# vwxyzjn/cleanrl

Measured on NVIDIA H100. Metric: env steps/sec (SPS) PPO Breakout num_envs=1024, higher is better.
Workload: dtype bf16

## Files before the change

cleanrl_b200/csrc/net_impala_tc.cu:

```cuda
#include <cuda.h>
#include <algorithm>
#include <cstring>
#include "tc_base.cuh"
#include "tc_gemm_tma.cuh"
#include "tc_reduce.cuh"
#include "tc_heads.cuh"
#include "tc_mma_sync.cuh"

namespace b200rl {
using namespace tc;

namespace imp {

constexpr int kThreads = 256;
constexpr int kWgradCtas = 264;

__device__ __forceinline__ float bf_lo(uint32_t w) { return __uint_as_float(w << 16); }
__device__ __forceinline__ float bf_hi(uint32_t w) { return __uint_as_float(w & 0xFFFF0000u); }
__device__ __forceinline__ uint32_t relu2(uint32_t w) {
    const uint32_t neg = ((w >> 15) & 0x00010001u) * 0xFFFFu;
    return w & ~neg;
}

struct Geo {
// ... 658 lines not shown
    float* wssmall = reinterpret_cast<float*>(reinterpret_cast<uint8_t*>(workspace) + impala_big_bytes());
    int rc;
    {
        ProfScope ps(s, "heads_bwd", 4.0 * n * 256 * A1, (double)n * (1024 + 8 * A1));
        if ((rc = heads_bwd_weight<256>(dhead, T(Q.hid), n, A1, wssmall, grads + L.hw, grads + L.hb, s, "impala/heads_bwd"))) return rc;
        if ((rc = heads_bwd_data<256>(dhead, params + L.hw, ab + Q.mhid, n, A1, T(Q.dhid), s, "impala/heads_bwd",
                                      values == 2 ? A : -1))) return rc;
    }
    {
        ProfScope ps(s, "fc_wgrad", 2.0 * n * 256 * 2048, (double)n * (2048 + 256) * 2 + 256.0 * 2048 * 4);
        const int splits = launch_wgrad_tma(T(Q.dhid), 256, T(Q.h0), 2048, n, wsbig, s, "impala/fc_wgrad");
        if (splits < 0) return splits;
        tc_fold_fc<<<2048, 256, 0, s>>>(wsbig, splits, 256, 2048, 256, 2048, 32, 64, 1.f, grads + L.fcw);
        if ((rc = check_launch("impala/fc_fold"))) return rc;
        if ((rc = colsum(T(Q.dhid), n, 256, 256, wssmall, grads + L.fcb, s))) return rc;
    }
    {
        KGemmParams g;
        memset(&g, 0, sizeof(g));
        g.scale = 1.f; g.A = T(Q.dhid); g.M = n; g.nchunks = 4;
        g.Bw = P + L.pfcd; g.N = 2048; g.out = T(Q.ga); g.ldo = 2048;
        g.mask_bits = reinterpret_cast<const uint32_t*>(ab + Q.mh0);
        ProfScope ps(s, "fc_dgrad", 2.0 * n * 256 * 2048, (double)n * (2048 + 256) * 2 + 256.0 * 2048 * 2);
        if ((rc = launch_gemm_tma<128, 4>(g, s, "impala/fc_dgrad"))) return rc;
    }
    bf16* G = T(Q.ga);
    bf16* Gn = T(Q.gb);
    const int cin[3] = {3, 16, 32}, cout[3] = {16, 32, 32};
    for (int q = 2; q >= 0; --q) {
        const int H = kH[q], OH = H / 2, C = cout[q], k0 = q * 5;
        for (int blk = 1; blk >= 0; --blk) {
            const int kc0 = k0 + 1 + 2 * blk, kc1 = kc0 + 1;
            bf16* x = T(Q.s[q][blk]);
            bf16* y0 = T(Q.y[q][blk]);
            ProfScope ps(s, "impala_res_bwd", 4 * 2.0 * n * OH * OH * C * 9 * C, 0);
            WgradP w1 = wgrad_defaults(geo(OH), wsbig, wssmall);
            w1.x = y0; w1.dy = G;
            ConvP d1 = conv_defaults(geo(OH));
            d1.in = G; d1.w = P + L.pd[kc1]; d1.epi = E_DGRAD; d1.aux = y0; d1.out = T(Q.gy);
            WgradP w0 = wgrad_defaults(geo(OH), wsbig, wssmall);
            w0.x = x; w0.relu_in = 1; w0.dy = T(Q.gy);
            ConvP d0 = conv_defaults(geo(OH));
            d0.in = T(Q.gy); d0.w = P + L.pd[kc0]; d0.epi = E_DGRAD; d0.aux = x; d0.skipg = G; d0.out = Gn;
            if (C == 16) {
                if ((rc = run_wgrad<16, 16>(w1, n, 1.f, grads + L.cw[kc1], grads + L.cb[kc1], s, "impala/res_wgrad1"))) return rc;
                if ((rc = run_conv<16, 16>(d1, n, s, "impala/res_dgrad1"))) return rc;
                if ((rc = run_wgrad<16, 16>(w0, n, 1.f, grads + L.cw[kc0], grads + L.cb[kc0], s, "impala/res_wgrad0"))) return rc;
// ... 50 lines not shown
```

cleanrl_b200/csrc/net_tc.cu:

```cuda
#include <cuda.h>
#include <algorithm>
#include "tc_base.cuh"
#include "tc_conv_win.cuh"
#include "tc_conv1_u8.cuh"
#include "tc_gemm_tma.cuh"
#include "tc_wgrad_win.cuh"
#include "tc_reduce.cuh"
#include "tc_aux.cuh"
#include "tc_heads.cuh"
#include "tc_heads_wide.cuh"
#include "tc_lstm.cuh"

namespace b200rl {

struct NatureLayout {
    int A;
    int64_t c1w, c1b, c2w, c2b, c3w, c3b, fcw, fcb, hw, hb, total;
    int64_t w1f, w2f, w2dg, w3f, w3dg, wfcf, wfcdg, w1l, w1sc, packed_total;
    bool wide; int G; int64_t whf, whdg, hbp;
    int64_t wih, whh, bih, bhh, whhp;
    explicit NatureLayout(int A_) : A(A_), wih(-1), whh(-1), bih(-1), bhh(-1), whhp(-1) {
        int64_t o = 0;
        c1w = o; o += 32 * 4 * 8 * 8;  c1b = o; o += 32;
        c2w = o; o += 64 * 32 * 4 * 4; c2b = o; o += 64;
// ... 147 lines not shown
    return wide_dhead_bytes(n, L) + colsum_f32_ws(n, A1);
}

static int trunk_fwd(const NatureLayout& L, const NatureActs& Q, const float* params, const bf16* P, bf16* act, int64_t n,
                     cudaStream_t s) {
    int rc;
    KGemmParams p;
    WinParams wp;
    win_defaults(wp); win_conv2(wp, act + Q.act1, n);
    wp.Bw = P + L.w2f; wp.N = 64; wp.vH = 9; wp.vW = 9; wp.out_mode = WOUT_DENSE; wp.out = act + Q.act2;
    wp.bias = params + L.c2b; wp.relu = 1; wp.mask_out = reinterpret_cast<uint32_t*>(act + Q.m2);
    { ProfScope ps(s, "conv2_fwd", 2.0 * n * 81 * 64 * 512, (double)n * ((12800 + 5184) * 2 + 648));
      if ((rc = launch_conv_win_t<128, 2, 2, 4>(wp, s, "naturecnn/conv2"))) return rc; }
    win_defaults(wp); win_conv3(wp, act + Q.act2, n);
    wp.Bw = P + L.w3f; wp.N = 64; wp.vH = 7; wp.vW = 7; wp.out_mode = WOUT_DENSE; wp.out = act + Q.act3;
    wp.bias = params + L.c3b; wp.relu = 1; wp.mask_out = reinterpret_cast<uint32_t*>(act + Q.m3);
    { ProfScope ps(s, "conv3_fwd", 2.0 * n * 49 * 64 * 576, (double)n * ((5184 + 3136) * 2 + 392));
      if ((rc = launch_conv_win_t<128, 1, 4, 9>(wp, s, "naturecnn/conv3"))) return rc; }
    gemm_rowmajor(p, act + Q.act3, n, 49);
    p.Bw = P + L.wfcf; p.N = 512; p.out = act + Q.hid; p.ldo = 512; p.bias = params + L.fcb; p.relu = 1;
    p.mask_out = reinterpret_cast<uint32_t*>(act + Q.m4);
    { ProfScope ps(s, "fc_fwd", 2.0 * n * 512 * 3136, (double)n * (3136 + 512) * 2 + 512.0 * 3136 * 2);
      if (n <= 8192) { if ((rc = launch_gemm_tma<64, 6>(p, s, "naturecnn/fc"))) return rc; }
      else if ((rc = launch_gemm_tma<128, 4>(p, s, "naturecnn/fc"))) return rc; }
    return B200RL_OK;
}

static int trunk_bwd(const NatureLayout& L, const NatureActs& Q, const bf16* P, bf16* act, float* grads, int64_t n,
                     float* wsbig, float* wssmall, void* tail_ready_event, bool dact1_fused, cudaStream_t s) {
    int rc;
    KGemmParams p;
    {
        int splits;
        { ProfScope ps(s, "fc_wgrad", 2.0 * n * 512 * 3136, (double)n * (3136 + 512) * 2 + 512.0 * 3136 * 4);
          if ((splits = launch_wgrad_tma(act + Q.dhid, 512, act + Q.act3, 3136, n, wsbig, s, "naturecnn/fc_wgrad")) < 0) return splits; }
        { ProfScope ps(s, "wgrad_fold_bias", 0, 0);
          note_launches(1); tc_fold_fc<<<(unsigned)ceil_div((int64_t)512 * 3136, 256), 256, 0, s>>>(wsbig, splits, 512, 13 * 256, 512, 3136, 64, 49, 1.f, grads + L.fcw);
          if ((rc = colsum(act + Q.dhid, n, 512, 512, wssmall, grads + L.fcb, s))) return rc; }
        if (tail_ready_event) {
            cudaError_t e = cudaEventRecord(reinterpret_cast<cudaEvent_t>(tail_ready_event), s);
            if (e != cudaSuccess) return fail(B200RL_ERR_CUDA, "naturecnn_backward: cudaEventRecord: %s", cudaGetErrorString(e));
        }
        gemm_rowmajor(p, act + Q.dhid, n, 8);
        p.Bw = P + L.wfcdg; p.N = 3136; p.out = act + Q.dact3a; p.out2 = act + Q.dact3b; p.dual_dact3 = 1;
        p.ldo = 3136; p.mask_bits = reinterpret_cast<const uint32_t*>(act + Q.m3);
        { ProfScope ps(s, "fc_dgrad", 2.0 * n * 512 * 3136, (double)n * ((3136 + 512) * 2 + 392) + 512.0 * 3136 * 2);
          if ((rc = launch_gemm_tma<128, 4>(p, s, "naturecnn/fc_dgrad"))) return rc; }
    }
    WGradWinParams gw;
    WinParams wp;
    FoldWin fw;
    {
        wgw_defaults(gw);
        gw.X = act + Q.act2; gw.M = n * 81; gw.n = (int)n; gw.G = 81; gw.cpr = 1; gw.nslots = 10; gw.WRX = round8(128 + 20);
        for (int t = 0; t < 9; ++t) gw.shift[t] = (t / 3) * 9 + (t % 3);
        const int st[10] = {0, 1, 2, 3, 4, 5, 6, 7, 7, 8};
        for (int k = 0; k < 10; ++k) { gw.slot_tap[k] = st[k]; gw.slot_cc[k] = 0; }
        gw.Y = act + Q.dact3a; gw.ldy = 64; gw.ncolsY = 64;
        const WPlan pl = conv3_wgrad_plan(n);
        gw.rows_per_cta = pl.rows_per_cta; gw.ws = wsbig; gw.wsb = wssmall;
        { ProfScope ps(s, "conv3_wgrad", 2.0 * n * 49 * 64 * 576, (double)n * (5184 + 5184) * 2);
          if ((rc = launch_wgrad_win(gw, pl.splits, s, "naturecnn/conv3_wgrad"))) return rc; }
        memset(&fw, 0, sizeof(fw));
        fw.layer = 3; fw.S = pl.splits; fw.nslots = 10; fw.Cout = 64; fw.scale = 1.f; fw.bscale = 1.f;
        for (int k = 0; k < 10; ++k) { fw.slot_tap[k] = st[k]; fw.slot_skip[k] = (k == 8); }
        { ProfScope ps(s, "wgrad_fold_bias", 0, 0);
          fw.wsb = wssmall; fw.db = grads + L.c3b;
          tc_fold_win<<<(unsigned)ceil_div(640 * 64 + 64, 32), 256, 0, s>>>(wsbig, fw, grads + L.c3w);
          if ((rc = check_launch("naturecnn/conv3_fold"))) return rc; }
        win_defaults(wp);
// ... 28 lines not shown
        for (int a = 0; a < 2; ++a) for (int b = 0; b < 2; ++b) wp.shift[a * 2 + b] = (1 - a) * 11 + (1 - b);
        wp.WR = round8(128 + 12);
        wp.Bw = P + L.w2dg; wp.N = 128; wp.vH = 10; wp.vW = 10; wp.out_mode = WOUT_DACT1;
        wp.out = act + Q.dact1; wp.mask_bits = reinterpret_cast<const uint32_t*>(act + Q.m1);
        { ProfScope ps(s, "conv2_dgrad", 2.0 * n * 400 * 32 * 256, (double)n * ((7744 + 14112) * 2 + 1600));
          if ((rc = launch_conv_win<128, 1, 4, 4>(wp, s, "naturecnn/conv2_dgrad"))) return rc; }
    }
    return B200RL_OK;
}
static size_t trunk_big_bytes(int64_t n) {
    return std::max({wgrad_tma_bytes(n, 512, 3136), wgrad_win_bytes(conv3_wgrad_plan(n).splits, 10),
                     wgrad_win_bytes(conv2_wgrad_plan(n).splits, 8)});
}
static size_t trunk_small_bytes(int64_t n) {
    return std::max({colsum_ws(n, 512), wgrad_win_bias_bytes(conv3_wgrad_plan(n).splits),
                     wgrad_win_bias_bytes(conv2_wgrad_plan(n).splits)});
}

static int wide_head_fwd(const NatureLayout& L, const bf16* P, const bf16* hid, int64_t n, int A1, float* out, cudaStream_t s) {
    KGemmParams p;
    gemm_rowmajor(p, hid, n, 8);
    p.Bw = P + L.whf; p.N = L.G; p.bias = reinterpret_cast<const float*>(P + L.hbp);
    p.out_f32 = out; p.ldo = A1; p.ncols_f32 = A1;
    return launch_gemm_tma<128, 4>(p, s, "wide_heads");
}

static int wide_head_bwd(const NatureLayout& L, const bf16* P, const float* dhead, int64_t n, int A1, const bf16* hid, bf16* dhid,
                         const uint32_t* hid_bits, float* dW, float* db, float* wsbig, float* wssmall, cudaStream_t s) {
    int rc;
    KGemmParams p;
    bf16* dh16 = reinterpret_cast<bf16*>(wssmall);
    float* dbpart = reinterpret_cast<float*>(reinterpret_cast<char*>(wssmall) + wide_dhead_bytes(n, L));
    int cb = (int)ceil_div(n * L.G, 256); if (cb > num_sms() * 8) cb = num_sms() * 8;
    tc_head_dhead_bf16<<<cb, 256, 0, s>>>(dhead, n, A1, L.G, dh16);
    if ((rc = check_launch("wide_heads_dhead"))) return rc;
    if ((rc = colsum_f32(dhead, n, A1, dbpart, db, s))) return rc;
    const int splits = launch_wgrad_tma(dh16, L.G, hid, 512, n, wsbig, s, "wide_heads_wgrad");
    if (splits < 0) return splits;
    tc_fold_fc<<<(unsigned)ceil_div((int64_t)A1 * 512, 256), 256, 0, s>>>(wsbig, splits, L.G, 512, A1, 512, 512, 1, 1.f, dW);
    if ((rc = check_launch("wide_heads_wgrad"))) return rc;
    gemm_rowmajor(p, dh16, n, L.G / 64);
    p.Bw = P + L.whdg; p.N = 512; p.out = dhid; p.ldo = 512;
    p.mask_bits = hid_bits;
    if (n <= 8192) { if ((rc = launch_gemm_tma<64, 6>(p, s, "wide_heads_dgrad"))) return rc; }
    else if ((rc = launch_gemm_tma<128, 4>(p, s, "wide_heads_dgrad"))) return rc;
    return B200RL_OK;
}
}

extern "C" int64_t b200rl_naturecnn_param_count(int A) { return A >= 1 ? NatureLayout(A).total : -1; }
extern "C" int64_t b200rl_naturecnn_grad_tail_offset(int A) { return A >= 1 ? NatureLayout(A).fcw : -1; }
extern "C" size_t b200rl_naturecnn_bf16_packed_bytes(int A) { return head_ok(A) ? (size_t)NatureLayout(A).packed_total * 2 : 0; }
extern "C" size_t b200rl_naturecnn_bf16_acts_bytes(int64_t n, int obs_format) {
    return n >= 0 ? (size_t)NatureActs(n, obs_format == B200RL_OBS_U8_NCHW).total * 2 + 256 : 0;
}

extern "C" int b200rl_frames_to_s2d_bf16(const uint8_t* obs, const int64_t* rows, int64_t n, void* out, void* stream) {
    B200RL_REQUIRE(n >= 0, "frames_to_s2d: negative n");
    if (n == 0) return B200RL_OK;
    B200RL_REQUIRE(obs && out, "frames_to_s2d: null pointer");
    B200RL_REQUIRE(aligned(obs, 4) && aligned(out, 16), "frames_to_s2d: misaligned buffer");
    cudaStream_t s = (cudaStream_t)stream;
    ProfScope ps(s, "frames_to_s2d", 0, (double)n * 28224 * 3);
    tc_frames_to_s2d<<<(unsigned)ceil_div(n * 1764, 256), 256, 0, s>>>(obs, rows, n, reinterpret_cast<bf16*>(out));
    return check_launch("frames_to_s2d");
}

extern "C" int b200rl_frames_to_s2d_u8(const uint8_t* obs, const int64_t* rows, int64_t n, uint8_t* out_rm, uint8_t* out_cm, void* stream) {
// ... 367 lines not shown
```

cleanrl_b200/csrc/tc_common.cuh:

```cuda
#pragma once
#include <cuda_bf16.h>
#include <cstdint>
#include "tc_wgmma.cuh"

namespace b200rl { namespace tc {

__device__ __forceinline__ uint32_t smem_u32(const void* p) {
    return static_cast<uint32_t>(__cvta_generic_to_shared(p));
}

__device__ __forceinline__ void mbar_init(uint64_t* bar, uint32_t count) {
    asm volatile("mbarrier.init.shared::cta.b64 [%0], %1;" ::"r"(smem_u32(bar)), "r"(count) : "memory");
}
__device__ __forceinline__ void fence_barrier_init() {
    asm volatile("fence.mbarrier_init.release.cluster;" ::: "memory");
}
__device__ __forceinline__ bool mbar_try_wait(uint64_t* bar, uint32_t parity) {
    uint32_t ok;
    asm volatile(
        "{\n\t.reg .pred p;\n\t"
        "mbarrier.try_wait.parity.shared::cta.b64 p, [%1], %2;\n\t"
        "selp.u32 %0, 1, 0, p;\n\t}\n"
        : "=r"(ok)
        : "r"(smem_u32(bar)), "r"(parity)
// ... 71 lines not shown

__device__ __forceinline__ uint32_t pack_bf16x2_relu(float lo, float hi) {
    uint32_t d;
    asm("cvt.rn.relu.bf16x2.f32 %0, %1, %2;" : "=r"(d) : "f"(hi), "f"(lo));
    return d;
}
__device__ __forceinline__ uint32_t pack_bf16x2(float lo, float hi) {
    __nv_bfloat162 v = __floats2bfloat162_rn(lo, hi);
    return *reinterpret_cast<uint32_t*>(&v);
}

}}

namespace b200rl { namespace tc {
__device__ __forceinline__ void cp_async16(uint32_t smem_addr, const void* gptr, uint32_t src_bytes) {
    asm volatile("cp.async.cg.shared.global [%0], [%1], 16, %2;" ::"r"(smem_addr), "l"(gptr), "r"(src_bytes) : "memory");
}
__device__ __forceinline__ void cp_async_commit() { asm volatile("cp.async.commit_group;" ::: "memory"); }
template <int N>
__device__ __forceinline__ void cp_async_wait() { asm volatile("cp.async.wait_group %0;" ::"n"(N) : "memory"); }
__device__ __forceinline__ void mbar_arrive(uint64_t* bar) {
    asm volatile("mbarrier.arrive.shared::cta.b64 _, [%0];" ::"r"(smem_u32(bar)) : "memory");
}
}}

namespace b200rl { namespace tc {
__device__ __forceinline__ void tma_load_2d(uint32_t smem_dst, const void* tmap, int x, int y, uint64_t* bar) {
    asm volatile("cp.async.bulk.tensor.2d.shared::cluster.global.mbarrier::complete_tx::bytes [%0], [%1, {%2, %3}], [%4];"
                 ::"r"(smem_dst), "l"(reinterpret_cast<uint64_t>(tmap)), "r"(x), "r"(y), "r"(smem_u32(bar))
                 : "memory");
}
__device__ __forceinline__ void tma_load_3d(uint32_t smem_dst, const void* tmap, int x, int y, int z, uint64_t* bar) {
    asm volatile("cp.async.bulk.tensor.3d.shared::cluster.global.mbarrier::complete_tx::bytes [%0], [%1, {%2, %3, %4}], [%5];"
                 ::"r"(smem_dst), "l"(reinterpret_cast<uint64_t>(tmap)), "r"(x), "r"(y), "r"(z), "r"(smem_u32(bar))
                 : "memory");
}
__device__ __forceinline__ void mbar_arrive_expect_tx(uint64_t* bar, uint32_t bytes) {
    asm volatile("mbarrier.arrive.expect_tx.shared::cta.b64 _, [%0], %1;" ::"r"(smem_u32(bar)), "r"(bytes) : "memory");
}
__device__ __forceinline__ void tma_prefetch_desc(const void* tmap) {
    asm volatile("prefetch.tensormap [%0];" ::"l"(reinterpret_cast<uint64_t>(tmap)) : "memory");
}
}}
```

cleanrl_b200/csrc/tc_conv1_u8.cuh:

```cuda
#pragma once
#include "tc_base.cuh"
#include <cuda_fp16.h>
#include "tc_conv_win.cuh"

namespace b200rl {
using namespace tc;

__device__ __forceinline__ uint64_t desc_kmajor_sw64(uint32_t smem_addr) {
    return (uint64_t)((smem_addr & 0x3FFFFu) >> 4) | (1ull << 16) | (32ull << 32) | kDescSwizzle64;
}
__device__ __forceinline__ uint64_t desc_mnmajor_sw64(uint32_t smem_addr, uint32_t lbo) {
    return (uint64_t)((smem_addr & 0x3FFFFu) >> 4) | ((uint64_t)((lbo >> 4) & 0x3FFF) << 16) | (32ull << 32) | kDescSwizzle64;
}
__device__ __forceinline__ uint32_t img64_off(int r, int c) { return (uint32_t)(r * 64 + ((c ^ ((r >> 1) & 3)) << 4)); }
__global__ void __launch_bounds__(256) tc_frames_to_s2d_u8(const uint8_t* __restrict__ obs, const int64_t* __restrict__ rows, int64_t n,
                                                           uint8_t* __restrict__ out_rm, uint8_t* __restrict__ out_cm) {
    __shared__ __align__(16) uint8_t plane[7056];
    const int64_t i = blockIdx.x >> 2;
    const int c = blockIdx.x & 3;
    const int64_t img = rows ? rows[i] : i;
    const int4* src = reinterpret_cast<const int4*>(obs + img * 28224 + c * 7056);
    for (int t = threadIdx.x; t < 441; t += 256) reinterpret_cast<int4*>(plane)[t] = __ldg(src + t);
    __syncthreads();
    for (int pos = threadIdx.x; pos < 441; pos += 256) {
// ... 207 lines not shown
    const uint32_t hi = up ? w[j + 2] : w[j + 1];
    return prmt(prmt(lo, hi, sel), 0x64646464u, 0x5140u);
}
__device__ __forceinline__ uint4 lds128(uint32_t addr) {
    uint4 v;
    asm volatile("ld.shared.v4.u32 {%0, %1, %2, %3}, [%4];" : "=r"(v.x), "=r"(v.y), "=r"(v.z), "=r"(v.w) : "r"(addr) : "memory");
    return v;
}
__device__ __forceinline__ uint32_t pack_f16x2_sat(float lo, float hi) {
    uint32_t d;
    asm("cvt.rn.satfinite.f16x2.f32 %0, %1, %2;" : "=r"(d) : "f"(hi), "f"(lo));
    return d;
}

__device__ __forceinline__ void sts32(uint32_t addr, uint32_t v) { asm volatile("st.shared.u32 [%0], %1;" ::"r"(addr), "r"(v) : "memory"); }
__device__ __forceinline__ void tma_store_3d(const void* tmap, uint32_t smem_src, int x, int y, int z) {
    asm volatile("cp.async.bulk.tensor.3d.global.shared::cta.bulk_group [%0, {%1, %2, %3}], [%4];"
                 ::"l"(reinterpret_cast<uint64_t>(tmap)), "r"(x), "r"(y), "r"(z), "r"(smem_src) : "memory");
}
__device__ __forceinline__ void bulk_commit() { asm volatile("cp.async.bulk.commit_group;" ::: "memory"); }
template <int N> __device__ __forceinline__ void bulk_wait_read() { asm volatile("cp.async.bulk.wait_group.read %0;" ::"n"(N) : "memory"); }
template <int N> __device__ __forceinline__ void bulk_wait() { asm volatile("cp.async.bulk.wait_group %0;" ::"n"(N) : "memory"); }

template <int R> __device__ __forceinline__ void setmaxnreg_dec() { asm volatile("setmaxnreg.dec.sync.aligned.u32 %0;" ::"n"(R)); }
template <int R> __device__ __forceinline__ void setmaxnreg_inc() { asm volatile("setmaxnreg.inc.sync.aligned.u32 %0;" ::"n"(R)); }
constexpr int kC1WRegsProducer = 40, kC21RegsDgrad = 128, kC1WRegsMma = 168;
static_assert(128 * kC1WRegsProducer + 128 * kC21RegsDgrad + 256 * kC1WRegsMma <= 65536, "register budgets exceed the SM");

constexpr int kC1WThreads = 512;
__global__ void __launch_bounds__(kC1WThreads, 1) tc_conv21_bwd_u8(const __grid_constant__ CUtensorMap tmX, const __grid_constant__ CUtensorMap tmWin,
                                                                 const __grid_constant__ CUtensorMap tmY, const Conv21BwdU8Params p) {
    constexpr int XS = kC1WXStages, WS = kC21WinStages;
    extern __shared__ uint8_t smem_raw[];
    __shared__ uint64_t xfull[XS], xempty[XS], wfull[WS], wempty[WS], yfull[2], yempty[2];
    __shared__ float sRed[32 * 32], sBias[32];
    uint8_t* smem = reinterpret_cast<uint8_t*>((reinterpret_cast<uintptr_t>(smem_raw) + 1023) & ~uintptr_t(1023));
    uint8_t* sW2 = smem;
    uint8_t* sWin = sW2 + kC21W2Bytes;
    uint8_t* sX = sWin + (size_t)WS * kC21WinBytes;
    uint8_t* sImg = sX + (size_t)XS * kC1WBlock;
    const int tid = threadIdx.x, warp = tid >> 5, lane = tid & 31;
    if (tid == 0) {
        for (int s = 0; s < XS; ++s) { mbar_init(&xfull[s], 1); mbar_init(&xempty[s], 12); }
        for (int s = 0; s < WS; ++s) { mbar_init(&wfull[s], 1); mbar_init(&wempty[s], 4); }
        for (int s = 0; s < 2; ++s) { mbar_init(&yfull[s], 1); mbar_init(&yempty[s], 8); }
        fence_barrier_init();
        tma_prefetch_desc(&tmX);
        tma_prefetch_desc(&tmWin);
// ... 237 lines not shown
```

cleanrl_b200/csrc/tc_gemm_tma.cuh:

```cuda
#pragma once
#include "tc_base.cuh"

namespace b200rl {
using namespace tc;

struct KGemmParams {
    const void* A;
    int64_t M;
    int nchunks;
    const bf16* Bw;
    int N;
    bf16* out;
    int ldo;
    const float* bias;
    float scale;
    int relu;
    const uint32_t* mask_bits;
    uint32_t* mask_out;
    int dual_dact3;
    bf16* out2;
    float* out_f32;
    int ncols_f32;
};

constexpr int kGemmThreads = 384;
template <int BN>
__host__ __device__ constexpr size_t gemm_acc_bytes() { return (size_t)128 * (BN + 4) * sizeof(float); }
template <int BN, int STAGES>
__global__ void __launch_bounds__(kGemmThreads, 1) tc_gemm_tma(const __grid_constant__ CUtensorMap tmA,
                                                               const __grid_constant__ CUtensorMap tmB,
                                                               const KGemmParams p, int total_tiles, int ntiles_n) {
    constexpr int A_BYTES = 128 * 128;
    constexpr int B_BYTES = BN * 128;
    constexpr int STAGE_BYTES = A_BYTES + B_BYTES;
    constexpr int LDA = BN + 4;
    extern __shared__ uint8_t smem_raw[];
    __shared__ uint64_t full_bar[STAGES], empty_bar[STAGES];
    uint8_t* smem = reinterpret_cast<uint8_t*>((reinterpret_cast<uintptr_t>(smem_raw) + 1023) & ~uintptr_t(1023));
    float* sAcc = reinterpret_cast<float*>(smem + (size_t)STAGES * STAGE_BYTES);
    const int tid = threadIdx.x, warp = tid >> 5;
    const int nch = p.nchunks;
    if (tid == 0) {
        for (int s = 0; s < STAGES; ++s) { mbar_init(&full_bar[s], 1); mbar_init(&empty_bar[s], 256); }
        fence_barrier_init();
        tma_prefetch_desc(&tmA);
        tma_prefetch_desc(&tmB);
    }
    __syncthreads();

    if (warp == 0) {
        if ((tid & 31) == 0) {
            uint32_t q = 0;
            for (int tile = blockIdx.x; tile < total_tiles; tile += gridDim.x) {
                const int mt = tile / ntiles_n, n0 = (tile - mt * ntiles_n) * BN;
                for (int j = 0; j < nch; ++j, ++q) {
                    const uint32_t s = q % STAGES;
                    if (q >= (uint32_t)STAGES) mbar_wait(&empty_bar[s], ((q / STAGES) - 1) & 1);
                    const uint32_t dst = smem_u32(smem + (size_t)s * STAGE_BYTES);
                    mbar_arrive_expect_tx(&full_bar[s], STAGE_BYTES);
                    tma_load_2d(dst, &tmA, j * 64, mt * 128, &full_bar[s]);
                    tma_load_2d(dst + A_BYTES, &tmB, j * 64, n0, &full_bar[s]);
                }
            }
        }
    } else if (warp >= 4) {
        const int wg = (warp - 4) >> 2, wt = tid & 127;
        float* st = sAcc + wg * 64 * LDA;
        const int lr = wt & 63, half = wt >> 6;
        const int nwords = p.N >> 5;
        constexpr int NW = BN / 32;
        float d[BN / 2];
#pragma unroll
        for (int e = 0; e < BN / 2; ++e) d[e] = 0.f;
        uint32_t q = 0;
        for (int tile = blockIdx.x; tile < total_tiles; tile += gridDim.x) {
            const int mt = tile / ntiles_n, n0 = (tile - mt * ntiles_n) * BN;
            for (int j = 0; j < nch; ++j, ++q) {
                const uint32_t s = q % STAGES;
                mbar_wait(&full_bar[s], (q / STAGES) & 1);
                wgmma_fence();
                const uint32_t stage_addr = smem_u32(smem + (size_t)s * STAGE_BYTES);
                const uint64_t a = desc_kmajor(stage_addr + wg * 64 * 128), b = desc_kmajor(stage_addr + A_BYTES);
#pragma unroll
                for (int kk = 0; kk < 4; ++kk) WgmmaBf16<BN, 0, 0>::mma(d, a + 2 * kk, b + 2 * kk, (j | kk) != 0 ? 1u : 0u);
                wgmma_commit();
                wgmma_wait<0>();
                mbar_arrive(&empty_bar[s]);
            }
            wgmma_fence_operands(d);
            const int r = mt * 128 + wg * 64 + lr;
            const bool rvalid = r < (int)p.M;
            const int64_t wb = (int64_t)r * nwords + (n0 >> 5);
            named_bar(1 + wg, 128);
            stage_acc(st, LDA, wt, d);
            named_bar(1 + wg, 128);
#pragma unroll
            for (int g = 0; g < NW; ++g) {
                const int col = n0 + g * 32;
                if (!rvalid || (g & 1) != half || col >= p.N) continue;
                uint32_t v[32];
#pragma unroll
                for (int e = 0; e < 8; ++e) {
                    const float4 f = *reinterpret_cast<const float4*>(st + lr * LDA + g * 32 + 4 * e);
                    v[4 * e] = __float_as_uint(f.x); v[4 * e + 1] = __float_as_uint(f.y);
                    v[4 * e + 2] = __float_as_uint(f.z); v[4 * e + 3] = __float_as_uint(f.w);
                }
                const uint32_t mbw = p.mask_bits != nullptr ? __ldg(p.mask_bits + wb + g) : 0xFFFFFFFFu;
                if (p.bias) {
                    const float4* bp = reinterpret_cast<const float4*>(p.bias + col);
#pragma unroll
                    for (int e = 0; e < 8; ++e) {
                        const float4 bv = __ldg(bp + e);
                        v[4 * e] = __float_as_uint(fmaf(__uint_as_float(v[4 * e]), p.scale, bv.x));
                        v[4 * e + 1] = __float_as_uint(fmaf(__uint_as_float(v[4 * e + 1]), p.scale, bv.y));
                        v[4 * e + 2] = __float_as_uint(fmaf(__uint_as_float(v[4 * e + 2]), p.scale, bv.z));
                        v[4 * e + 3] = __float_as_uint(fmaf(__uint_as_float(v[4 * e + 3]), p.scale, bv.w));
                    }
                } else {
#pragma unroll
                    for (int e = 0; e < 32; ++e) v[e] = __float_as_uint(__uint_as_float(v[e]) * p.scale);
                }
                if (p.relu) {
                    uint32_t bits = 0u;
#pragma unroll
                    for (int e = 0; e < 32; ++e) {
                        const bool pos = __uint_as_float(v[e]) > 0.f;
                        bits |= (pos ? 1u : 0u) << e;
                        v[e] = pos ? v[e] : 0u;
                    }
                    if (p.mask_out) p.mask_out[wb + g] = bits;
                }
                if (p.mask_bits) {
#pragma unroll
                    for (int e = 0; e < 32; ++e) if (!((mbw >> e) & 1u)) v[e] = 0u;
                }
                if (p.out_f32) {
                    float* dst = p.out_f32 + (int64_t)r * p.ldo + col;
#pragma unroll
                    for (int e = 0; e < 32; ++e) if (col + e < p.ncols_f32) dst[e] = __uint_as_float(v[e]);
                    continue;
                }
                int4 w[4];
#pragma unroll
                for (int e = 0; e < 4; ++e) {
                    w[e].x = (int)pack_bf16x2(__uint_as_float(v[8 * e]), __uint_as_float(v[8 * e + 1]));
                    w[e].y = (int)pack_bf16x2(__uint_as_float(v[8 * e + 2]), __uint_as_float(v[8 * e + 3]));
                    w[e].z = (int)pack_bf16x2(__uint_as_float(v[8 * e + 4]), __uint_as_float(v[8 * e + 5]));
                    w[e].w = (int)pack_bf16x2(__uint_as_float(v[8 * e + 6]), __uint_as_float(v[8 * e + 7]));
                }
                if (p.dual_dact3) {
                    const int px = col >> 6;
                    const int oy = px / 7, ox = px - oy * 7;
                    bf16* dst = p.out + ((int64_t)r * 81 + oy * 9 + ox) * 64 + (g & 1) * 32;
                    bf16* dst2 = p.out2 + ((int64_t)r * 121 + (oy + 2) * 11 + ox + 2) * 64 + (g & 1) * 32;
                    st_global_32b(dst, w[0], w[1]); st_global_32b(dst + 16, w[2], w[3]);
                    st_global_32b(dst2, w[0], w[1]); st_global_32b(dst2 + 16, w[2], w[3]);
                } else {
                    bf16* dst = p.out + (int64_t)r * p.ldo + col;
                    st_global_32b(dst, w[0], w[1]); st_global_32b(dst + 16, w[2], w[3]);
                }
            }
        }
    }
}

constexpr int kWgradTmaThreads = 384;
constexpr int kFcWgradXChunks = 2, kFcWgradYChunks = 4;
static __global__ void __launch_bounds__(kWgradTmaThreads, 1) tc_wgrad_tma(const __grid_constant__ CUtensorMap tmX,
                                                                    const __grid_constant__ CUtensorMap tmY,
                                                                    int64_t M, int64_t rows_per_cta, float* ws) {
    constexpr int R = 64, STAGES = 4, nxc = kFcWgradXChunks, nyc = kFcWgradYChunks, NY = 64 * nyc;
    extern __shared__ uint8_t smem_raw[];
    __shared__ uint64_t full_bar[STAGES], empty_bar[STAGES];
    uint8_t* smem = reinterpret_cast<uint8_t*>((reinterpret_cast<uintptr_t>(smem_raw) + 1023) & ~uintptr_t(1023));
    const int tid = threadIdx.x, warp = tid >> 5;
    const int xc0 = blockIdx.y * nxc, yc0 = blockIdx.z * nyc;
    constexpr int chunk_img = R * 128;
    constexpr int stage_bytes = (nxc + nyc) * chunk_img;
    if (tid == 0) {
        for (int s = 0; s < STAGES; ++s) { mbar_init(&full_bar[s], 1); mbar_init(&empty_bar[s], 8); }
        fence_barrier_init();
        tma_prefetch_desc(&tmX);
        tma_prefetch_desc(&tmY);
    }
    __syncthreads();
    const int64_t m_begin = (int64_t)blockIdx.x * rows_per_cta;
    int64_t m_end = m_begin + rows_per_cta;
    if (m_end > M) m_end = M;
    const int nsteps = m_end > m_begin ? (int)((m_end - m_begin + R - 1) / R) : 0;

    if (warp == 0 && (tid & 31) == 0) {
        for (int it = 0; it < nsteps; ++it) {
            const int s = it % STAGES;
            if (it >= STAGES) mbar_wait(&empty_bar[s], ((it / STAGES) - 1) & 1);
            const uint32_t dst = smem_u32(smem + (size_t)s * stage_bytes);
            const int m0 = (int)(m_begin + (int64_t)it * R);
            mbar_arrive_expect_tx(&full_bar[s], (uint32_t)stage_bytes);
            for (int c = 0; c < nxc; ++c) tma_load_2d(dst + c * chunk_img, &tmX, (xc0 + c) * 64, m0, &full_bar[s]);
            for (int c = 0; c < nyc; ++c) tma_load_2d(dst + (nxc + c) * chunk_img, &tmY, (yc0 + c) * 64, m0, &full_bar[s]);
        }
    } else if (warp >= 4) {
        const int wg = (warp - 4) >> 2, wt = tid & 127;
        float d[NY / 2];
#pragma unroll
        for (int e = 0; e < NY / 2; ++e) d[e] = 0.f;
        for (int it = 0; it < nsteps; ++it) {
            const int s = it % STAGES;
            mbar_wait(&full_bar[s], (it / STAGES) & 1);
            wgmma_fence();
            const uint32_t xa = smem_u32(smem + (size_t)s * stage_bytes), ya = xa + nxc * chunk_img;
#pragma unroll
            for (int kk = 0; kk < R / 16; ++kk) {
                const uint64_t adesc = desc_mnmajor(xa + wg * chunk_img + kk * 2048, chunk_img);
                const uint64_t bdesc = desc_mnmajor(ya + kk * 2048, chunk_img);
                WgmmaBf16<NY, 1, 1>::mma(d, adesc, bdesc, (it | kk) != 0 ? 1u : 0u);
            }
            wgmma_commit();
            wgmma_wait<0>();
            if ((tid & 31) == 0) mbar_arrive(&empty_bar[s]);
        }
        wgmma_fence_operands(d);
        const int64_t NYtot = (int64_t)gridDim.z * nyc * 64;
        const int64_t KXtot = (int64_t)gridDim.y * nxc * 64;
        float* wsb = ws + (int64_t)blockIdx.x * KXtot * NYtot;
        const int row = ((wt >> 5) << 4) + ((wt & 31) >> 2), col = (wt & 3) * 2;
        float* d0 = wsb + ((int64_t)xc0 * 64 + wg * 64 + row) * NYtot + (int64_t)yc0 * 64 + col;
        float* d8 = d0 + 8 * NYtot;
#pragma unroll
        for (int j = 0; j < NY / 8; ++j) {
            *reinterpret_cast<float2*>(d0 + 8 * j) = make_float2(d[4 * j], d[4 * j + 1]);
            *reinterpret_cast<float2*>(d8 + 8 * j) = make_float2(d[4 * j + 2], d[4 * j + 3]);
        }
    }
}

template <int BN, int STAGES>
static int launch_gemm_tma(const KGemmParams& p, cudaStream_t s, const char* what) {
    const size_t smem = (size_t)STAGES * (128 * 128 + BN * 128) + gemm_acc_bytes<BN>() + 1024;
    static SmemAttrCache attr;
    int rc;
    if (p.N % 64 != 0 || BN % 64 != 0) return fail(B200RL_ERR_INVALID_ARGUMENT, "%s: N must be a multiple of 64", what);
    if ((rc = attr.ensure(tc_gemm_tma<BN, STAGES>, smem, what))) return rc;
    CUtensorMap tmA, tmB;
    const int64_t K = (int64_t)p.nchunks * 64;
    if ((rc = make_tmap_2d(&tmA, p.A, p.M, K, 128, what))) return rc;
    if ((rc = make_tmap_2d(&tmB, p.Bw, p.N, K, BN, what))) return rc;
    const int ntn = (int)ceil_div(p.N, BN);
    const int total = (int)ceil_div(p.M, 128) * ntn;
    int grid = num_sms();
    if (grid > total) grid = total;
    tc_gemm_tma<BN, STAGES><<<grid, kGemmThreads, smem, s>>>(tmA, tmB, p, total, ntn);
    return check_launch(what);
}

static int64_t round_up(int64_t a, int64_t b) { return ceil_div(a, b) * b; }
struct WPlan { int64_t rows_per_cta; int splits; };
static WPlan wgrad_plan(int64_t M, int target_ctas, int quantum = 32) {
    WPlan w;
    w.rows_per_cta = round_up(ceil_div(M, target_ctas), quantum);
    if (w.rows_per_cta < quantum) w.rows_per_cta = quantum;
    w.splits = (int)ceil_div(M, w.rows_per_cta);
    if (w.splits < 1) w.splits = 1;
    return w;
}
constexpr int kFcSplits = 8;

static size_t wgrad_tma_bytes(int64_t M, int xcols, int ycols) {
    return (size_t)wgrad_plan(M, kFcSplits, 64).splits * xcols * round_up(ycols, 64 * kFcWgradYChunks) * sizeof(float);
}
static int launch_wgrad_tma(const void* X, int xcols, const void* Y, int ycols, int64_t M, float* ws, cudaStream_t s,
                            const char* what) {
    if (xcols % (64 * kFcWgradXChunks) != 0) return fail(B200RL_ERR_INVALID_ARGUMENT, "%s: X columns must be a multiple of 128", what);
    const WPlan pl = wgrad_plan(M, kFcSplits, 64);
    CUtensorMap tmX, tmY;
    int rc;
    if ((rc = make_tmap_2d(&tmX, X, M, xcols, 64, what))) return rc;
    if ((rc = make_tmap_2d(&tmY, Y, M, ycols, 64, what))) return rc;
    const size_t smem = (size_t)4 * (kFcWgradXChunks + kFcWgradYChunks) * 64 * 128 + 1024;
    static SmemAttrCache attr;
    if ((rc = attr.ensure(tc_wgrad_tma, smem, what))) return rc;
    const dim3 grid(pl.splits, xcols / (64 * kFcWgradXChunks), (unsigned)ceil_div(ycols, 64 * kFcWgradYChunks));
    tc_wgrad_tma<<<grid, kWgradTmaThreads, smem, s>>>(tmX, tmY, M, pl.rows_per_cta, ws);
    if ((rc = check_launch(what))) return rc;
    return pl.splits;
}

}
```

Before: 1.174 million.

## Restructure TMA GEMM into two independent warpgroup pipelines with register rebalancing

```diff
diff --git a/cleanrl_b200/csrc/net_impala_tc.cu b/cleanrl_b200/csrc/net_impala_tc.cu
--- a/cleanrl_b200/csrc/net_impala_tc.cu
+++ b/cleanrl_b200/csrc/net_impala_tc.cu
@@ -704,7 +704,7 @@
         g.Bw = P + L.pfcd; g.N = 2048; g.out = T(Q.ga); g.ldo = 2048;
         g.mask_bits = reinterpret_cast<const uint32_t*>(ab + Q.mh0);
         ProfScope ps(s, "fc_dgrad", 2.0 * n * 256 * 2048, (double)n * (2048 + 256) * 2 + 256.0 * 2048 * 2);
-        if ((rc = launch_gemm_tma<128, 4>(g, s, "impala/fc_dgrad"))) return rc;
+        if ((rc = launch_gemm_tma<128, 3>(g, s, "impala/fc_dgrad"))) return rc;
     }
     bf16* G = T(Q.ga);
     bf16* Gn = T(Q.gb);
diff --git a/cleanrl_b200/csrc/net_tc.cu b/cleanrl_b200/csrc/net_tc.cu
--- a/cleanrl_b200/csrc/net_tc.cu
+++ b/cleanrl_b200/csrc/net_tc.cu
@@ -193,7 +193,7 @@
     p.mask_out = reinterpret_cast<uint32_t*>(act + Q.m4);
     { ProfScope ps(s, "fc_fwd", 2.0 * n * 512 * 3136, (double)n * (3136 + 512) * 2 + 512.0 * 3136 * 2);
       if (n <= 8192) { if ((rc = launch_gemm_tma<64, 6>(p, s, "naturecnn/fc"))) return rc; }
-      else if ((rc = launch_gemm_tma<128, 4>(p, s, "naturecnn/fc"))) return rc; }
+      else if ((rc = launch_gemm_tma<128, 3>(p, s, "naturecnn/fc"))) return rc; }
     return B200RL_OK;
 }
 
@@ -216,7 +216,7 @@
         p.Bw = P + L.wfcdg; p.N = 3136; p.out = act + Q.dact3a; p.out2 = act + Q.dact3b; p.dual_dact3 = 1;
         p.ldo = 3136; p.mask_bits = reinterpret_cast<const uint32_t*>(act + Q.m3);
         { ProfScope ps(s, "fc_dgrad", 2.0 * n * 512 * 3136, (double)n * ((3136 + 512) * 2 + 392) + 512.0 * 3136 * 2);
-          if ((rc = launch_gemm_tma<128, 4>(p, s, "naturecnn/fc_dgrad"))) return rc; }
+          if ((rc = launch_gemm_tma<128, 3>(p, s, "naturecnn/fc_dgrad"))) return rc; }
     }
     WGradWinParams gw;
     WinParams wp;
@@ -291,7 +291,7 @@
     gemm_rowmajor(p, hid, n, 8);
     p.Bw = P + L.whf; p.N = L.G; p.bias = reinterpret_cast<const float*>(P + L.hbp);
     p.out_f32 = out; p.ldo = A1; p.ncols_f32 = A1;
-    return launch_gemm_tma<128, 4>(p, s, "wide_heads");
+    return launch_gemm_tma<128, 3>(p, s, "wide_heads");
 }
 
 static int wide_head_bwd(const NatureLayout& L, const bf16* P, const float* dhead, int64_t n, int A1, const bf16* hid, bf16* dhid,
@@ -312,7 +312,7 @@
     p.Bw = P + L.whdg; p.N = 512; p.out = dhid; p.ldo = 512;
     p.mask_bits = hid_bits;
     if (n <= 8192) { if ((rc = launch_gemm_tma<64, 6>(p, s, "wide_heads_dgrad"))) return rc; }
-    else if ((rc = launch_gemm_tma<128, 4>(p, s, "wide_heads_dgrad"))) return rc;
+    else if ((rc = launch_gemm_tma<128, 3>(p, s, "wide_heads_dgrad"))) return rc;
     return B200RL_OK;
 }
 }
diff --git a/cleanrl_b200/csrc/tc_common.cuh b/cleanrl_b200/csrc/tc_common.cuh
--- a/cleanrl_b200/csrc/tc_common.cuh
+++ b/cleanrl_b200/csrc/tc_common.cuh
@@ -117,6 +117,8 @@
 __device__ __forceinline__ void mbar_arrive(uint64_t* bar) {
     asm volatile("mbarrier.arrive.shared::cta.b64 _, [%0];" ::"r"(smem_u32(bar)) : "memory");
 }
+template <int R> __device__ __forceinline__ void setmaxnreg_dec() { asm volatile("setmaxnreg.dec.sync.aligned.u32 %0;" ::"n"(R)); }
+template <int R> __device__ __forceinline__ void setmaxnreg_inc() { asm volatile("setmaxnreg.inc.sync.aligned.u32 %0;" ::"n"(R)); }
 }}
 
 namespace b200rl { namespace tc {
diff --git a/cleanrl_b200/csrc/tc_conv1_u8.cuh b/cleanrl_b200/csrc/tc_conv1_u8.cuh
--- a/cleanrl_b200/csrc/tc_conv1_u8.cuh
+++ b/cleanrl_b200/csrc/tc_conv1_u8.cuh
@@ -253,8 +253,6 @@
 template <int N> __device__ __forceinline__ void bulk_wait_read() { asm volatile("cp.async.bulk.wait_group.read %0;" ::"n"(N) : "memory"); }
 template <int N> __device__ __forceinline__ void bulk_wait() { asm volatile("cp.async.bulk.wait_group %0;" ::"n"(N) : "memory"); }
 
-template <int R> __device__ __forceinline__ void setmaxnreg_dec() { asm volatile("setmaxnreg.dec.sync.aligned.u32 %0;" ::"n"(R)); }
-template <int R> __device__ __forceinline__ void setmaxnreg_inc() { asm volatile("setmaxnreg.inc.sync.aligned.u32 %0;" ::"n"(R)); }
 constexpr int kC1WRegsProducer = 40, kC21RegsDgrad = 128, kC1WRegsMma = 168;
 static_assert(128 * kC1WRegsProducer + 128 * kC21RegsDgrad + 256 * kC1WRegsMma <= 65536, "register budgets exceed the SM");
 
diff --git a/cleanrl_b200/csrc/tc_gemm_tma.cuh b/cleanrl_b200/csrc/tc_gemm_tma.cuh
--- a/cleanrl_b200/csrc/tc_gemm_tma.cuh
+++ b/cleanrl_b200/csrc/tc_gemm_tma.cuh
@@ -24,144 +24,219 @@
 };
 
 constexpr int kGemmThreads = 384;
+constexpr int kGemmRegsProducer = 40, kGemmRegsMma = 232;
+static_assert(128 * kGemmRegsProducer + 256 * kGemmRegsMma <= 65536, "register budgets exceed the SM");
 template <int BN>
-__host__ __device__ constexpr size_t gemm_acc_bytes() { return (size_t)128 * (BN + 4) * sizeof(float); }
+__host__ __device__ constexpr size_t gemm_acc_bytes() { return (size_t)8 * 8 * (BN + 4) * sizeof(float); }
+
+template <int BN, int STAGES>
+__device__ __forceinline__ void gemm_tile_mma(float (&d)[BN / 64][BN / 2], uint32_t ring, uint64_t* full_bar,
+                                              uint64_t* empty_bar, uint32_t q0, int nch, int tid) {
+    constexpr int MH = BN / 64;
+    constexpr int A_BYTES = BN * 128;
+    constexpr int STAGE_BYTES = A_BYTES + BN * 128;
+    auto chunk = [&](int j) {
+        const uint32_t q = q0 + (uint32_t)j, s = q % STAGES;
+        mbar_wait(&full_bar[s], (q / STAGES) & 1);
+        wgmma_fence();
+        const uint32_t stage_addr = ring + s * STAGE_BYTES;
+        const uint64_t b = desc_kmajor(stage_addr + A_BYTES);
+#pragma unroll
+        for (int h = 0; h < MH; ++h) {
+            const uint64_t a = desc_kmajor(stage_addr + h * 64 * 128);
+#pragma unroll
+            for (int kk = 0; kk < 4; ++kk) WgmmaBf16<BN, 0, 0>::mma(d[h], a + 2 * kk, b + 2 * kk, (j | kk) != 0 ? 1u : 0u);
+        }
+        wgmma_commit();
+    };
+    for (int j = 0; j + 1 < nch; ++j) {
+        chunk(j);
+        wgmma_wait<1>();
+        if (j > 0 && (tid & 31) == 0) mbar_arrive(&empty_bar[(q0 + (uint32_t)j - 1u) % STAGES]);
+    }
+    chunk(nch - 1);
+    wgmma_wait<0>();
+#pragma unroll
+    for (int h = 0; h < MH; ++h) wgmma_fence_operands(d[h]);
+    if ((tid & 31) == 0) {
+        if (nch > 1) mbar_arrive(&empty_bar[(q0 + (uint32_t)nch - 2u) % STAGES]);
+        mbar_arrive(&empty_bar[(q0 + (uint32_t)nch - 1u) % STAGES]);
+    }
+}
+
 template <int BN, int STAGES>
 __global__ void __launch_bounds__(kGemmThreads, 1) tc_gemm_tma(const __grid_constant__ CUtensorMap tmA,
                                                                const __grid_constant__ CUtensorMap tmB,
                                                                const KGemmParams p, int total_tiles, int ntiles_n) {
-    constexpr int A_BYTES = 128 * 128;
-    constexpr int B_BYTES = BN * 128;
-    constexpr int STAGE_BYTES = A_BYTES + B_BYTES;
+    static_assert(BN == 64 || BN == 128, "one epilogue lane per row and 32-column group of 8 rows");
+    constexpr int MH = BN / 64;
+    constexpr int A_BYTES = BN * 128;
+    constexpr int STAGE_BYTES = A_BYTES + BN * 128;
     constexpr int LDA = BN + 4;
+    constexpr int NW = BN / 32;
+    constexpr int PR = BN / 8;
     extern __shared__ uint8_t smem_raw[];
-    __shared__ uint64_t full_bar[STAGES], empty_bar[STAGES];
+    __shared__ uint64_t full_bar[2][STAGES], empty_bar[2][STAGES];
     uint8_t* smem = reinterpret_cast<uint8_t*>((reinterpret_cast<uintptr_t>(smem_raw) + 1023) & ~uintptr_t(1023));
-    float* sAcc = reinterpret_cast<float*>(smem + (size_t)STAGES * STAGE_BYTES);
-    const int tid = threadIdx.x, warp = tid >> 5;
+    float* sAcc = reinterpret_cast<float*>(smem + (size_t)2 * STAGES * STAGE_BYTES);
+    const int tid = threadIdx.x, warp = tid >> 5, lane = tid & 31;
     const int nch = p.nchunks;
     if (tid == 0) {
-        for (int s = 0; s < STAGES; ++s) { mbar_init(&full_bar[s], 1); mbar_init(&empty_bar[s], 256); }
+        for (int w = 0; w < 2; ++w)
+            for (int s = 0; s < STAGES; ++s) { mbar_init(&full_bar[w][s], 1); mbar_init(&empty_bar[w][s], 4); }
         fence_barrier_init();
         tma_prefetch_desc(&tmA);
         tma_prefetch_desc(&tmB);
     }
     __syncthreads();
 
-    if (warp == 0) {
-        if ((tid & 31) == 0) {
+    if (warp < 4) {
+        setmaxnreg_dec<kGemmRegsProducer>();
+        if (warp < 2 && lane == 0) {
+            const int w = warp;
+            uint8_t* ring = smem + (size_t)w * STAGES * STAGE_BYTES;
             uint32_t q = 0;
-            for (int tile = blockIdx.x; tile < total_tiles; tile += gridDim.x) {
+            for (int tile = blockIdx.x + w * gridDim.x; tile < total_tiles; tile += 2 * gridDim.x) {
                 const int mt = tile / ntiles_n, n0 = (tile - mt * ntiles_n) * BN;
                 for (int j = 0; j < nch; ++j, ++q) {
                     const uint32_t s = q % STAGES;
-                    if (q >= (uint32_t)STAGES) mbar_wait(&empty_bar[s], ((q / STAGES) - 1) & 1);
-                    const uint32_t dst = smem_u32(smem + (size_t)s * STAGE_BYTES);
-                    mbar_arrive_expect_tx(&full_bar[s], STAGE_BYTES);
-                    tma_load_2d(dst, &tmA, j * 64, mt * 128, &full_bar[s]);
-                    tma_load_2d(dst + A_BYTES, &tmB, j * 64, n0, &full_bar[s]);
+                    if (q >= (uint32_t)STAGES) mbar_wait(&empty_bar[w][s], ((q / STAGES) - 1) & 1);
+                    const uint32_t dst = smem_u32(ring + (size_t)s * STAGE_BYTES);
+                    mbar_arrive_expect_tx(&full_bar[w][s], STAGE_BYTES);
+                    tma_load_2d(dst, &tmA, j * 64, mt * BN, &full_bar[w][s]);
+                    tma_load_2d(dst + A_BYTES, &tmB, j * 64, n0, &full_bar[w][s]);
                 }
             }
         }
-    } else if (warp >= 4) {
-        const int wg = (warp - 4) >> 2, wt = tid & 127;
-        float* st = sAcc + wg * 64 * LDA;
-        const int lr = wt & 63, half = wt >> 6;
+    } else {
+        setmaxnreg_inc<kGemmRegsMma>();
+        const int wg = (warp - 4) >> 2, ww = (warp - 4) & 3;
+        float* st = sAcc + (warp - 4) * 8 * LDA;
+        const uint32_t ring = smem_u32(smem + (size_t)wg * STAGES * STAGE_BYTES);
         const int nwords = p.N >> 5;
-        constexpr int NW = BN / 32;
-        float d[BN / 2];
-#pragma unroll
-        for (int e = 0; e < BN / 2; ++e) d[e] = 0.f;
+        const int er = lane & 7, eg = lane >> 3;
         uint32_t q = 0;
-        for (int tile = blockIdx.x; tile < total_tiles; tile += gridDim.x) {
+        for (int tile = blockIdx.x + wg * gridDim.x; tile < total_tiles; tile += 2 * gridDim.x, q += (uint32_t)nch) {
             const int mt = tile / ntiles_n, n0 = (tile - mt * ntiles_n) * BN;
-            for (int j = 0; j < nch; ++j, ++q) {
-                const uint32_t s = q % STAGES;
-                mbar_wait(&full_bar[s], (q / STAGES) & 1);
-                wgmma_fence();
-                const uint32_t stage_addr = smem_u32(smem + (size_t)s * STAGE_BYTES);
-                const uint64_t a = desc_kmajor(stage_addr + wg * 64 * 128), b = desc_kmajor(stage_addr + A_BYTES);
-#pragma unroll
-                for (int kk = 0; kk < 4; ++kk) WgmmaBf16<BN, 0, 0>::mma(d, a + 2 * kk, b + 2 * kk, (j | kk) != 0 ? 1u : 0u);
-                wgmma_commit();
-                wgmma_wait<0>();
-                mbar_arrive(&empty_bar[s]);
+            float d[MH][BN / 2];
+#pragma unroll
+            for (int h = 0; h < MH; ++h)
+#pragma unroll
+                for (int e = 0; e < BN / 2; ++e) d[h][e] = 0.f;
+            gemm_tile_mma<BN, STAGES>(d, ring, full_bar[wg], empty_bar[wg], q, nch, tid);
+#pragma unroll
+            for (int pass = 0; pass < 2 * MH; ++pass) {
+                const int h = pass >> 1, hi = pass & 1;
+                const int row0 = mt * BN + 64 * h + 16 * ww + 8 * hi;
+#pragma unroll
+                for (int j = 0; j < BN / 8; ++j)
+                    *reinterpret_cast<float2*>(st + (lane >> 2) * LDA + 8 * j + 2 * (lane & 3)) =
+                        make_float2(d[h][4 * j + 2 * hi], d[h][4 * j + 2 * hi + 1]);
+                __syncwarp();
+                const int r = row0 + er, col = n0 + eg * 32;
+                const bool live = eg < NW && r < (int)p.M && col < p.N;
+                int4 w[4];
+                if (live) {
+                    const int64_t wb = (int64_t)r * nwords + (col >> 5);
+                    uint32_t v[32];
+#pragma unroll
+                    for (int e = 0; e < 8; ++e) {
+                        const float4 f = *reinterpret_cast<const float4*>(st + er * LDA + eg * 32 + 4 * e);
+                        v[4 * e] = __float_as_uint(f.x); v[4 * e + 1] = __float_as_uint(f.y);
+                        v[4 * e + 2] = __float_as_uint(f.z); v[4 * e + 3] = __float_as_uint(f.w);
+                    }
+                    const uint32_t mbw = p.mask_bits != nullptr ? __ldg(p.mask_bits + wb) : 0xFFFFFFFFu;
+                    if (p.bias) {
+                        const float4* bp = reinterpret_cast<const float4*>(p.bias + col);
+#pragma unroll
+                        for (int e = 0; e < 8; ++e) {
+                            const float4 bv = __ldg(bp + e);
+                            v[4 * e] = __float_as_uint(fmaf(__uint_as_float(v[4 * e]), p.scale, bv.x));
+                            v[4 * e + 1] = __float_as_uint(fmaf(__uint_as_float(v[4 * e + 1]), p.scale, bv.y));
+                            v[4 * e + 2] = __float_as_uint(fmaf(__uint_as_float(v[4 * e + 2]), p.scale, bv.z));
+                            v[4 * e + 3] = __float_as_uint(fmaf(__uint_as_float(v[4 * e + 3]), p.scale, bv.w));
+                        }
+                    } else {
+#pragma unroll
+                        for (int e = 0; e < 32; ++e) v[e] = __float_as_uint(__uint_as_float(v[e]) * p.scale);
+                    }
+                    if (p.relu) {
+                        uint32_t bits = 0u;
+#pragma unroll
+                        for (int e = 0; e < 32; ++e) {
+                            const bool pos = __uint_as_float(v[e]) > 0.f;
+                            bits |= (pos ? 1u : 0u) << e;
+                            v[e] = pos ? v[e] : 0u;
+                        }
+                        if (p.mask_out) p.mask_out[wb] = bits;
+                    }
+                    if (p.mask_bits) {
+#pragma unroll
+                        for (int e = 0; e < 32; ++e) if (!((mbw >> e) & 1u)) v[e] = 0u;
+                    }
+                    if (p.out_f32) {
+                        float* dst = p.out_f32 + (int64_t)r * p.ldo + col;
+#pragma unroll
+                        for (int e = 0; e < 32; ++e) if (col + e < p.ncols_f32) dst[e] = __uint_as_float(v[e]);
+                    }
+#pragma unroll
+                    for (int e = 0; e < 4; ++e) {
+                        w[e].x = (int)pack_bf16x2(__uint_as_float(v[8 * e]), __uint_as_float(v[8 * e + 1]));
+                        w[e].y = (int)pack_bf16x2(__uint_as_float(v[8 * e + 2]), __uint_as_float(v[8 * e + 3]));
+                        w[e].z = (int)pack_bf16x2(__uint_as_float(v[8 * e + 4]), __uint_as_float(v[8 * e + 5]));
+                        w[e].w = (int)pack_bf16x2(__uint_as_float(v[8 * e + 6]), __uint_as_float(v[8 * e + 7]));
+                    }
+                }
+                __syncwarp();
+                if (live) {
+                    int4* brow = reinterpret_cast<int4*>(st + er * LDA) + 4 * eg;
+#pragma unroll
+                    for (int e = 0; e < 4; ++e) brow[e] = w[e];
+                }
+                __syncwarp();
+                if (p.out_f32 == nullptr) {
+#pragma unroll
+                    for (int k = lane; k < 8 * PR; k += 32) {
+                        const int rr = k / PR, pc = k % PR;
+                        const int rs = row0 + rr, cs = n0 + pc * 8;
+                        if (rs >= (int)p.M || cs >= p.N) continue;
+                        const int4 val = reinterpret_cast<const int4*>(st + rr * LDA)[pc];
+                        if (p.dual_dact3) {
+                            const int px = cs >> 6;
+                            const int oy = px / 7, ox = px - oy * 7;
+                            *reinterpret_cast<int4*>(p.out + ((int64_t)rs * 81 + oy * 9 + ox) * 64 + (cs & 63)) = val;
+                            *reinterpret_cast<int4*>(p.out2 + ((int64_t)rs * 121 + (oy + 2) * 11 + ox + 2) * 64 + (cs & 63)) = val;
+                        } else {
+                            *reinterpret_cast<int4*>(p.out + (int64_t)rs * p.ldo + cs) = val;
+                        }
+                    }
+                }
+                __syncwarp();
             }
-            wgmma_fence_operands(d);
-            const int r = mt * 128 + wg * 64 + lr;
-            const bool rvalid = r < (int)p.M;
-            const int64_t wb = (int64_t)r * nwords + (n0 >> 5);
-            named_bar(1 + wg, 128);
-            stage_acc(st, LDA, wt, d);
-            named_bar(1 + wg, 128);
-#pragma unroll
-            for (int g = 0; g < NW; ++g) {
-                const int col = n0 + g * 32;
-                if (!rvalid || (g & 1) != half || col >= p.N) continue;
-                uint32_t v[32];
-#pragma unroll
-                for (int e = 0; e < 8; ++e) {
-                    const float4 f = *reinterpret_cast<const float4*>(st + lr * LDA + g * 32 + 4 * e);
-                    v[4 * e] = __float_as_uint(f.x); v[4 * e + 1] = __float_as_uint(f.y);
-                    v[4 * e + 2] = __float_as_uint(f.z); v[4 * e + 3] = __float_as_uint(f.w);
-                }
-                const uint32_t mbw = p.mask_bits != nullptr ? __ldg(p.mask_bits + wb + g) : 0xFFFFFFFFu;
-                if (p.bias) {
-                    const float4* bp = reinterpret_cast<const float4*>(p.bias + col);
-#pragma unroll
-                    for (int e = 0; e < 8; ++e) {
-                        const float4 bv = __ldg(bp + e);
-                        v[4 * e] = __float_as_uint(fmaf(__uint_as_float(v[4 * e]), p.scale, bv.x));
-                        v[4 * e + 1] = __float_as_uint(fmaf(__uint_as_float(v[4 * e + 1]), p.scale, bv.y));
-                        v[4 * e + 2] = __float_as_uint(fmaf(__uint_as_float(v[4 * e + 2]), p.scale, bv.z));
-                        v[4 * e + 3] = __float_as_uint(fmaf(__uint_as_float(v[4 * e + 3]), p.scale, bv.w));
-                    }
-                } else {
-#pragma unroll
-                    for (int e = 0; e < 32; ++e) v[e] = __float_as_uint(__uint_as_float(v[e]) * p.scale);
-                }
-                if (p.relu) {
-                    uint32_t bits = 0u;
-#pragma unroll
-                    for (int e = 0; e < 32; ++e) {
-                        const bool pos = __uint_as_float(v[e]) > 0.f;
-                        bits |= (pos ? 1u : 0u) << e;
-                        v[e] = pos ? v[e] : 0u;
-                    }
-                    if (p.mask_out) p.mask_out[wb + g] = bits;
-                }
-                if (p.mask_bits) {
-#pragma unroll
-                    for (int e = 0; e < 32; ++e) if (!((mbw >> e) & 1u)) v[e] = 0u;
-                }
-                if (p.out_f32) {
-                    float* dst = p.out_f32 + (int64_t)r * p.ldo + col;
-#pragma unroll
-                    for (int e = 0; e < 32; ++e) if (col + e < p.ncols_f32) dst[e] = __uint_as_float(v[e]);
-                    continue;
-                }
-                int4 w[4];
-#pragma unroll
-                for (int e = 0; e < 4; ++e) {
-                    w[e].x = (int)pack_bf16x2(__uint_as_float(v[8 * e]), __uint_as_float(v[8 * e + 1]));
-                    w[e].y = (int)pack_bf16x2(__uint_as_float(v[8 * e + 2]), __uint_as_float(v[8 * e + 3]));
-                    w[e].z = (int)pack_bf16x2(__uint_as_float(v[8 * e + 4]), __uint_as_float(v[8 * e + 5]));
-                    w[e].w = (int)pack_bf16x2(__uint_as_float(v[8 * e + 6]), __uint_as_float(v[8 * e + 7]));
-                }
-                if (p.dual_dact3) {
-                    const int px = col >> 6;
-                    const int oy = px / 7, ox = px - oy * 7;
-                    bf16* dst = p.out + ((int64_t)r * 81 + oy * 9 + ox) * 64 + (g & 1) * 32;
-                    bf16* dst2 = p.out2 + ((int64_t)r * 121 + (oy + 2) * 11 + ox + 2) * 64 + (g & 1) * 32;
-                    st_global_32b(dst, w[0], w[1]); st_global_32b(dst + 16, w[2], w[3]);
-                    st_global_32b(dst2, w[0], w[1]); st_global_32b(dst2 + 16, w[2], w[3]);
-                } else {
-                    bf16* dst = p.out + (int64_t)r * p.ldo + col;
-                    st_global_32b(dst, w[0], w[1]); st_global_32b(dst + 16, w[2], w[3]);
-                }
-            }
-        }
-    }
+        }
+    }
+}
+
+template <int BN, int STAGES>
+static int launch_gemm_tma(const KGemmParams& p, cudaStream_t s, const char* what) {
+    const size_t smem = (size_t)2 * STAGES * (BN * 128 + BN * 128) + gemm_acc_bytes<BN>() + 1024;
+    static SmemAttrCache attr;
+    int rc;
+    if (p.N % 64 != 0 || BN % 64 != 0) return fail(B200RL_ERR_INVALID_ARGUMENT, "%s: N must be a multiple of 64", what);
+    if (p.nchunks < 1) return fail(B200RL_ERR_INVALID_ARGUMENT, "%s: K must be at least 64", what);
+    if (p.out_f32 == nullptr && !p.dual_dact3 && p.ldo % 8 != 0)
+        return fail(B200RL_ERR_INVALID_ARGUMENT, "%s: output pitch must be a multiple of 8 (16-byte stores)", what);
+    if ((rc = attr.ensure(tc_gemm_tma<BN, STAGES>, smem, what))) return rc;
+    CUtensorMap tmA, tmB;
+    const int64_t K = (int64_t)p.nchunks * 64;
+    if ((rc = make_tmap_2d(&tmA, p.A, p.M, K, BN, what))) return rc;
+    if ((rc = make_tmap_2d(&tmB, p.Bw, p.N, K, BN, what))) return rc;
+    const int ntn = (int)ceil_div(p.N, BN);
+    const int total = (int)ceil_div(p.M, BN) * ntn;
+    int grid = num_sms();
+    if (grid > total) grid = total;
+    tc_gemm_tma<BN, STAGES><<<grid, kGemmThreads, smem, s>>>(tmA, tmB, p, total, ntn);
+    return check_launch(what);
 }
 
 constexpr int kWgradTmaThreads = 384;
@@ -204,7 +279,7 @@
         float d[NY / 2];
 #pragma unroll
         for (int e = 0; e < NY / 2; ++e) d[e] = 0.f;
-        for (int it = 0; it < nsteps; ++it) {
+        auto step = [&](int it) {
             const int s = it % STAGES;
             mbar_wait(&full_bar[s], (it / STAGES) & 1);
             wgmma_fence();
@@ -216,9 +291,14 @@
                 WgmmaBf16<NY, 1, 1>::mma(d, adesc, bdesc, (it | kk) != 0 ? 1u : 0u);
             }
             wgmma_commit();
-            wgmma_wait<0>();
-            if ((tid & 31) == 0) mbar_arrive(&empty_bar[s]);
-        }
+        };
+        for (int it = 0; it + 1 < nsteps; ++it) {
+            step(it);
+            wgmma_wait<1>();
+            if (it > 0 && (tid & 31) == 0) mbar_arrive(&empty_bar[(it - 1) % STAGES]);
+        }
+        step(nsteps - 1);
+        wgmma_wait<0>();
         wgmma_fence_operands(d);
         const int64_t NYtot = (int64_t)gridDim.z * nyc * 64;
         const int64_t KXtot = (int64_t)gridDim.y * nxc * 64;
@@ -232,25 +312,6 @@
             *reinterpret_cast<float2*>(d8 + 8 * j) = make_float2(d[4 * j + 2], d[4 * j + 3]);
         }
     }
-}
-
-template <int BN, int STAGES>
-static int launch_gemm_tma(const KGemmParams& p, cudaStream_t s, const char* what) {
-    const size_t smem = (size_t)STAGES * (128 * 128 + BN * 128) + gemm_acc_bytes<BN>() + 1024;
-    static SmemAttrCache attr;
-    int rc;
-    if (p.N % 64 != 0 || BN % 64 != 0) return fail(B200RL_ERR_INVALID_ARGUMENT, "%s: N must be a multiple of 64", what);
-    if ((rc = attr.ensure(tc_gemm_tma<BN, STAGES>, smem, what))) return rc;
-    CUtensorMap tmA, tmB;
-    const int64_t K = (int64_t)p.nchunks * 64;
-    if ((rc = make_tmap_2d(&tmA, p.A, p.M, K, 128, what))) return rc;
-    if ((rc = make_tmap_2d(&tmB, p.Bw, p.N, K, BN, what))) return rc;
-    const int ntn = (int)ceil_div(p.N, BN);
-    const int total = (int)ceil_div(p.M, 128) * ntn;
-    int grid = num_sms();
-    if (grid > total) grid = total;
-    tc_gemm_tma<BN, STAGES><<<grid, kGemmThreads, smem, s>>>(tmA, tmB, p, total, ntn);
-    return check_launch(what);
 }
 
 static int64_t round_up(int64_t a, int64_t b) { return ceil_div(a, b) * b; }
@@ -272,6 +333,11 @@
                             const char* what) {
     if (xcols % (64 * kFcWgradXChunks) != 0) return fail(B200RL_ERR_INVALID_ARGUMENT, "%s: X columns must be a multiple of 128", what);
     const WPlan pl = wgrad_plan(M, kFcSplits, 64);
+    if (M < 1) {
+        const cudaError_t e = cudaMemsetAsync(ws, 0, wgrad_tma_bytes(M, xcols, ycols), s);
+        if (e != cudaSuccess) return fail(B200RL_ERR_CUDA, "%s: cudaMemsetAsync: %s", what, cudaGetErrorString(e));
+        return pl.splits;
+    }
     CUtensorMap tmX, tmY;
     int rc;
     if ((rc = make_tmap_2d(&tmX, X, M, xcols, 64, what))) return rc;
```

Result: faster. 1.223 million (median of 6 runs) (+4.2%).
